# Plachtaa/FAcodec

Measured on NVIDIA B200. Metric: audio_seconds_per_second, higher is better.
Workload: dtype f32 I/O and accumulation; every product is a 3-MMA split of fp32 operands: fp16 hi + 2^11-scaled fp16 lo (22 mantissa bits, register-promoted accumulation) upstream of the VQ, bf16 hi + bf16 lo (16 bits) downstream

## Files before the change

facodec_b200/csrc/conv_tt.cu:

```cuda
#include <cstring>
#include <mutex>

#include "common.cuh"
#include "conv_tc_common.cuh"
#include "kernels.h"

namespace fac {

namespace tc {
constexpr int kThreadsT = 512;
constexpr int kProdT = 192;
constexpr int kStagesT = 4;
constexpr int kABufT = 4;
constexpr int kPfT = 3;
constexpr int kMT = 128;
constexpr int kAccT = 128;
struct SmemT {
    uint64_t b_full[kStagesT];
    uint64_t b_empty[kStagesT];
    uint64_t a_full[kABufT];
    uint64_t a_empty[kABufT];
    uint64_t acc_ready;
    uint64_t acc_free;
    uint32_t tmem_base;
    uint32_t pad;
};
static_assert(sizeof(SmemT) <= kSmemHdr, "SmemT header");
}

__device__ __forceinline__ float sin2_wide(float x) {
    const double kd = rint((double)x * 0.31830988618379067154);
    const float r = (float)fma(-kd, 3.14159265358979323846, (double)x);
    const float r2 = r * r;
    float q = fmaf(r2, 1.60590438368216146e-10f, -2.50521083854417188e-8f);
    q = fmaf(q, r2, 2.75573192239858907e-6f);
    q = fmaf(q, r2, -1.98412698412698413e-4f);
    q = fmaf(q, r2, 8.33333333333333333e-3f);
    q = fmaf(q, r2, -1.66666666666666667e-1f);
    q = fmaf(q * r2, r, r);
    return q * q;
}
__device__ __forceinline__ float4 snake4_w(float4 x, float4 al, float4 ia) {
    const float y0 = al.x * x.x, y1 = al.y * x.y, y2 = al.z * x.z, y3 = al.w * x.w;
    const float m = fmaxf(fmaxf(fabsf(y0), fabsf(y1)), fmaxf(fabsf(y2), fabsf(y3)));
    float4 o;
    if (m > 4096.0f) {
// ... 102 lines not shown
    const int pc = ptid & 3;
    const int r0 = ptid >> 2;
    const bool has_alpha = p.in_alpha != nullptr;
    const bool mufu = p.snake_mufu != 0;
    float4 al = make_float4(0.f, 0.f, 0.f, 0.f), ia = al;
    if (has_alpha) {
        const int j = c * tc::kChunk + pc * 4;
        const int ci = j - (j / p.Cin) * p.Cin;
        al = __ldg(reinterpret_cast<const float4*>(p.in_alpha + ci));
        ia = __ldg(reinterpret_cast<const float4*>(p.in_inv_alpha + ci));
    }
    const uint32_t off0 = ((uint32_t)(pc >> 1) * Rpad + r0) * 16 + (uint32_t)(pc & 1) * 8;
    const float4* __restrict__ st = reinterpret_cast<const float4*>(stage) + ptid;
#pragma unroll
    for (int u = 0; u < NB; ++u) {
        if (r0 + u * RSTEP < R) {
            float4 x4 = st[u * NTHR];
            if (has_alpha) x4 = mufu ? snake4_mufu(x4, al, ia) : snake4_w(x4, al, ia);
            split_store_h(x4, ahi, alo, off0 + u * (RSTEP * 16));
        }
    }
}

template <int ACTT>
__device__ __forceinline__ void epilogue_slab8(float (&v)[8], float bi, float al, float ia, int act, float* __restrict__ yb,
                                               const float* __restrict__ rb, uint32_t off, uint32_t ldy, int nvalid, bool mufu) {
    float r[8];
    if (rb) {
#pragma unroll
        for (int i = 0; i < 8; ++i) r[i] = (i < nvalid) ? rb[off + i * ldy] : 0.f;
    }
#pragma unroll
    for (int i = 0; i < 8; ++i) v[i] += bi;
    if (ACTT == ACT_SNAKE || (ACTT < 0 && act == ACT_SNAKE)) {
        float y[8], m = 0.f;
#pragma unroll
        for (int i = 0; i < 8; ++i) { y[i] = al * v[i]; m = fmaxf(m, fabsf(y[i])); }
        if (m > 4096.0f) {
#pragma unroll
            for (int i = 0; i < 8; ++i) v[i] = fmaf(ia, sin2_wide(y[i]), v[i]);
        } else if (mufu) {
#pragma unroll
            for (int i = 0; i < 8; ++i) v[i] = fmaf(ia, sin2_mufu(y[i]), v[i]);
        } else {
#pragma unroll
            for (int i = 0; i < 8; ++i) v[i] = fmaf(ia, sin2_poly(y[i]), v[i]);
        }
    } else if (ACTT < 0 && act == ACT_TANH) {
#pragma unroll 1
        for (int i = 0; i < 8; ++i) v[i] = tanhf(v[i]);
    } else if (ACTT < 0 && act == ACT_MISH) {
#pragma unroll 1
        for (int i = 0; i < 8; ++i) v[i] = mish_f(v[i]);
    }
    if (rb) {
#pragma unroll
        for (int i = 0; i < 8; ++i) v[i] += r[i];
    }
    if (nvalid >= 8) {
#pragma unroll
        for (int i = 0; i < 8; ++i) yb[off + i * ldy] = v[i];
    } else {
#pragma unroll
        for (int i = 0; i < 8; ++i)
            if (i < nvalid) yb[off + i * ldy] = v[i];
    }
}

__device__ long long g_tt_probe[8];

template <bool PROBE, int ACTT>
__global__ void __launch_bounds__(tc::kThreadsT, 1) conv_tt_kernel(TcConvParams p) {
    using namespace tc;
    extern __shared__ __align__(128) uint8_t smem_raw[];
    SmemT* sm = reinterpret_cast<SmemT*>(smem_raw);
    constexpr int KG = 2;
    const int NT = p.NT;
    const int R = NT + (p.Kr - 1) * p.dil;
    const int Rpad = p.Rpad;
    const uint32_t a_half = (uint32_t)Rpad * 16 * KG;
    constexpr uint32_t w_half = (uint32_t)kMT * 16 * KG;
    uint8_t* a_base = smem_raw + kSmemHdr;
    uint8_t* w_base = a_base + (size_t)kABufT * 2 * a_half;
    const int CT = p.pair ? 2 : 1;
    const uint32_t w_stage = (uint32_t)CT * 2 * w_half;
    uint8_t* stg_base = w_base + (size_t)kStagesT * w_stage;
    constexpr int S = kStagesT;
    const int P = p.promote_every;

    const int tid = threadIdx.x, warp = tid >> 5, lane = tid & 31;
    const int nchunk = p.nchunk, Kr = p.Kr;
    const int gx = (p.Tout + NT - 1) / NT, gy = ((p.Cout + kMT - 1) / kMT) / CT;
    const int ntiles = gx * gy * p.B;
    const int G = (nchunk + P - 1) / P;

    if (tid == 0) {
        for (int i = 0; i < S; ++i) { mbar_init(&sm->b_full[i], 1); mbar_init(&sm->b_empty[i], 1); }
        for (int i = 0; i < kABufT; ++i) { mbar_init(&sm->a_full[i], kProdT); mbar_init(&sm->a_empty[i], 1); }
        mbar_init(&sm->acc_ready, 1);
        mbar_init(&sm->acc_free, 256);
        fence_mbar_init();
    }
    constexpr int kWarpTma = 14, kWarpMma = 15;
    if (warp == kWarpMma) tmem_alloc(&sm->tmem_base, 512);
    tc_fence_before();
    __syncthreads();
    tc_fence_after();
    const uint32_t tmem = sm->tmem_base;

    if (warp >= 8) reg_dec<64>();
    if (warp == kWarpTma) {
        if (lane == 0) {
            int it = 0;
            for (int L = blockIdx.x; L < ntiles; L += gridDim.x) {
                const int ntile = (L % gy) * CT;
                const size_t tile_floats = (size_t)nchunk * Kr * (size_t)(2 * w_half / 4);
                const float* wsrc = p.wblob + (size_t)ntile * tile_floats;
                for (int j = 0; j < nchunk * Kr; ++j, ++it) {
                    const int s = it % S;
                    mbar_wait_park<200>(&sm->b_empty[s], ((it / S) & 1) ^ 1);
                    mbar_arrive_expect_tx(&sm->b_full[s], w_stage);
                    for (int ct = 0; ct < CT; ++ct)
                        bulk_g2s(w_base + (size_t)s * w_stage + (size_t)ct * 2 * w_half, wsrc + (size_t)ct * tile_floats + (size_t)j * (2 * w_half / 4),
                                 2 * w_half, &sm->b_full[s]);
                }
            }
        }
    } else if (warp == kWarpMma) {
        const uint32_t idesc = (1u << 4) | ((uint32_t)(NT >> 3) << 17) | ((128u >> 4) << 24);
        const uint32_t tmem_u = __shfl_sync(0xffffffffu, tmem, 0);
        const uint32_t a_base16 = __shfl_sync(0xffffffffu, smem_u32(a_base), 0) >> 4;
        const uint32_t w_base16 = __shfl_sync(0xffffffffu, smem_u32(w_base), 0) >> 4;
        const uint32_t a_lbo16 = (uint32_t)Rpad, w_lbo16 = (uint32_t)kMT;
        const uint32_t a_half16 = a_half >> 4, w_half16 = w_half >> 4;
        const uint32_t d0 = tmem_u, d1 = tmem_u + 256u;
        int it = 0, cg = 0, gg = 0;
        const bool mprobe = PROBE && blockIdx.x == 3;
        long long w_a = 0, w_b = 0, w_acc = 0, tq = 0;
        for (int L = blockIdx.x; L < ntiles; L += gridDim.x) {
            for (int g = 0; g < G; ++g, ++gg) {
                if (mprobe) tq = clock64();
                mbar_wait(&sm->acc_free, (gg & 1) ^ 1);
                if (mprobe) w_acc += clock64() - tq;
                tc_fence_after();
                const int c_begin = g * P, c_end = (c_begin + P < nchunk) ? c_begin + P : nchunk;
                for (int c = c_begin; c < c_end; ++c, ++cg) {
                    const int buf = cg % kABufT;
                    if (mprobe) tq = clock64();
                    mbar_wait(&sm->a_full[buf], (cg / kABufT) & 1);
                    if (mprobe) w_a += clock64() - tq;
                    const uint32_t x_hi = a_base16 + (uint32_t)buf * 2 * a_half16;
                    const uint32_t x_lo = x_hi + a_half16;
                    for (int tap = 0; tap < Kr; ++tap, ++it) {
                        const int s = it % S;
                        if (mprobe) tq = clock64();
                        mbar_wait(&sm->b_full[s], (it / S) & 1);
                        if (mprobe) w_b += clock64() - tq;
                        tc_fence_after();
                        const uint32_t row_off = (uint32_t)(tap * p.dil);
                        const uint32_t first0 = ((c - c_begin) | tap) != 0, first1 = (g | (c - c_begin) | tap) != 0;
                        for (int ct = 0; ct < CT; ++ct) {
                            const uint32_t w_hi = w_base16 + (uint32_t)s * (w_stage >> 4) + (uint32_t)ct * 2 * w_half16;
                            const uint32_t w_lo = w_hi + w_half16;
                            const uint32_t dc = (uint32_t)ct * 128u;
                            umma_bf16(d0 + dc, desc_u(w_hi, w_lbo16), desc_u(x_hi + row_off, a_lbo16), idesc, first0);
                            umma_bf16(d1 + dc, desc_u(w_hi, w_lbo16), desc_u(x_lo + row_off, a_lbo16), idesc, first1);
                            umma_bf16(d1 + dc, desc_u(w_lo, w_lbo16), desc_u(x_hi + row_off, a_lbo16), idesc, 1u);
                        }
                        umma_commit(&sm->b_empty[s]);
                    }
                    umma_commit(&sm->a_empty[buf]);
                }
                umma_commit(&sm->acc_ready);
            }
        }
        if (mprobe && lane == 0) { g_tt_probe[2] = w_a; g_tt_probe[3] = w_b; g_tt_probe[4] = w_acc; }
    } else if (warp >= 8) {
        const int wtid = tid - 256;
        const PadMap pm = PadMap::make(p.Tin, p.pad_left_s, p.pad_right_s, p.reflect);
        const bool pprobe = PROBE && blockIdx.x == 3 && wtid == 0;
        const long long t_start = pprobe ? clock64() : 0;
        long long w_ae = 0, tq = 0;
        struct Cur { int L, c, t0, vrow0; bool interior; const float* xb; };
        auto setup = [&](Cur& k) {
            k.t0 = ((k.L / gy) % gx) * NT;
            k.xb = p.x + (size_t)(k.L / (gx * gy)) * p.x_bstride;
            k.vrow0 = k.t0 - p.PLr;
            k.interior = k.vrow0 >= 0 && (k.vrow0 + R) * p.vf <= p.Tin && k.t0 + NT <= p.Tout && R <= 7 * (kProdT / 4);
        };
        auto advance = [&](Cur& k) {
            if (++k.c == nchunk) { k.c = 0; k.L += gridDim.x; if (k.L < ntiles) setup(k); }
        };
        Cur pf{(int)blockIdx.x, 0, 0, 0, false, nullptr}, cs = pf;
        if (pf.L < ntiles) { setup(pf); cs = pf; }
        constexpr uint32_t kStageBytes = 7u * kProdT * 16u;
#pragma unroll 1
        for (int i = 0; i < kPfT - 1; ++i) {
// ... 9 lines not shown
            if (pf.L < ntiles) {
                if (pf.interior) stage_chunk_interior<kProdT, 7>(p, pf.xb, pf.c, pf.vrow0, R, stg_base + (size_t)((cg + kPfT - 1) % kPfT) * kStageBytes, wtid);
                advance(pf);
            }
            cp_async_commit_tt();
            cp_async_wait_tt<kPfT - 1>();
            const int buf = cg % kABufT;
            uint8_t* ahi = a_base + (size_t)buf * 2 * a_half;
            if (pprobe) tq = clock64();
            mbar_wait_park<200>(&sm->a_empty[buf], ((cg / kABufT) & 1) ^ 1);
            if (pprobe) w_ae += clock64() - tq;
            if (cs.interior) transform_chunk_interior<kProdT, 7>(p, cs.c, R, Rpad, stg_base + (size_t)(cg % kPfT) * kStageBytes, ahi, ahi + a_half, wtid);
            else produce_chunk_edge<kProdT>(p, pm, cs.xb, cs.c, cs.t0, R, Rpad, ahi, ahi + a_half, wtid);
            fence_proxy_async();
            mbar_arrive(&sm->a_full[buf]);
            advance(cs);
        }
        cp_async_wait_tt<0>();
        if (pprobe) { g_tt_probe[0] = clock64() - t_start; g_tt_probe[1] = w_ae; }
    } else {
        reg_inc<192>();
        const int q = warp & 3;
        const int half = warp >> 2;
        int split = ((NT / 2 + 15) / 16) * 16;
        if (split > NT) split = NT;
        const int mycol0 = CT == 2 ? half * 128 : (half ? split : 0);
        const int mytime0 = CT == 2 ? 0 : mycol0;
        const int mycols = CT == 2 ? NT : (half ? NT - split : split);
        const int act = p.out_act;
        int gg = 0;
        const bool aprobe = PROBE && blockIdx.x == 3 && tid == 0;
        long long w_ar = 0, t_dr = 0, t_ep = 0, tq = 0;
        for (int L = blockIdx.x; L < ntiles; L += gridDim.x) {
            const int ntile = (L % gy) * CT + (CT == 2 ? half : 0);
            const int t0 = ((L / gy) % gx) * NT;
            const int b = L / (gx * gy);
            const int co = ntile * kMT + q * 32 + lane;
            const bool co_ok = co < p.Cout;
            float acc[kAccT];
#pragma unroll
            for (int i = 0; i < kAccT; ++i) acc[i] = 0.f;
            for (int g = 0; g < G; ++g, ++gg) {
                if (aprobe) tq = clock64();
                mbar_wait_park<100>(&sm->acc_ready, gg & 1);
                if (aprobe) { long long n = clock64(); w_ar += n - tq; tq = n; }
                tc_fence_after();
                const uint32_t tb0 = tmem + ((uint32_t)(q * 32) << 16) + (uint32_t)mycol0;
#pragma unroll
                for (int grp = 0; grp < kAccT / 16; ++grp) {
                    if (grp * 16 < mycols) {
                        uint32_t v[16];
                        tmem_ld16(tb0 + grp * 16, v);
#pragma unroll
                        for (int i = 0; i < 16; ++i) acc[grp * 16 + i] += __uint_as_float(v[i]);
                    }
                }
                if (g == G - 1) {
#pragma unroll
                    for (int grp = 0; grp < kAccT / 16; ++grp) {
                        if (grp * 16 < mycols) {
                            uint32_t v[16];
                            tmem_ld16(tb0 + 256u + grp * 16, v);
#pragma unroll
                            for (int i = 0; i < 16; ++i) acc[grp * 16 + i] = fmaf(__uint_as_float(v[i]), kLoUnscale, acc[grp * 16 + i]);
                        }
                    }
                }
                tc_fence_before();
                mbar_arrive(&sm->acc_free);
                if (aprobe) t_dr += clock64() - tq;
            }
            if (aprobe) tq = clock64();
            float* __restrict__ yb = p.y + (size_t)b * p.y_bstride + co;
            const float* __restrict__ rb = p.res ? p.res + (size_t)b * p.y_bstride + co : nullptr;
            float bi = 0.f, al = 0.f, ia = 0.f;
            if (co_ok) {
                if (p.bias) bi = __ldg(p.bias + co);
                if (act == ACT_SNAKE) { al = __ldg(p.out_alpha + co); ia = __ldg(p.out_inv_alpha + co); }
            }
            const int tbeg = t0 + mytime0;
            const uint32_t ldy = (uint32_t)p.ldy;
#pragma unroll 1
            for (int sl = 0; sl * 8 < mycols; ++sl) {
                float v[8];
#define FAC_SLAB(S0) _Pragma("unroll") for (int i = 0; i < 8; ++i) v[i] = acc[(S0) + i];
                switch (sl) {
                    case 0: FAC_SLAB(0) break;
                    case 1: FAC_SLAB(8) break;
                    case 2: FAC_SLAB(16) break;
                    case 3: FAC_SLAB(24) break;
                    case 4: FAC_SLAB(32) break;
                    case 5: FAC_SLAB(40) break;
                    case 6: FAC_SLAB(48) break;
                    case 7: FAC_SLAB(56) break;
                    case 8: FAC_SLAB(64) break;
                    case 9: FAC_SLAB(72) break;
                    case 10: FAC_SLAB(80) break;
                    case 11: FAC_SLAB(88) break;
                    case 12: FAC_SLAB(96) break;
                    case 13: FAC_SLAB(104) break;
                    case 14: FAC_SLAB(112) break;
                    default: FAC_SLAB(120) break;
                }
#undef FAC_SLAB
                const int ts = tbeg + sl * 8;
                const int nvalid = co_ok ? p.Tout - ts : 0;
                if (nvalid > 0) epilogue_slab8<ACTT>(v, bi, al, ia, act, yb, rb, (uint32_t)ts * ldy, ldy, nvalid, p.snake_mufu != 0);
            }
            if (aprobe) t_ep += clock64() - tq;
        }
        if (aprobe) { g_tt_probe[5] = w_ar; g_tt_probe[6] = t_dr; g_tt_probe[7] = t_ep; }
    }
    tc_fence_before();
    __syncthreads();
    if (warp == kWarpMma) tmem_dealloc(tmem, 512);
}

int g_tt_pair_ok = 1;

bool tt_conv_plan(TcConvParams& p) {
    if ((p.Cin % 4) != 0 || ((p.Cin * p.vf) % tc::kChunk) != 0 || p.Cout < 1) return false;
    p.tt = 1; p.promoted = 1; p.f16x2 = 1; p.bf16 = 0; p.fused = 0;
    p.N = tc::kMT; p.MT = 1;
    p.nchunk = p.Cin * p.vf / tc::kChunk;
    p.nchunk2 = 0;
    int NT = 256;
    if (p.Tout > 0) {
        auto padded = [&](int nt) { return (long long)((p.Tout + nt - 1) / nt) * nt; };
        long long best = padded(256);
        for (int cand = 240; cand >= 128; cand -= 16)
            if (padded(cand) * 10 < best * 9) { best = padded(cand); NT = cand; }
    }
    const int ntile_co = (p.Cout + tc::kMT - 1) / tc::kMT;
    p.pair = (g_tt_pair_ok && p.Kr <= 3 && ntile_co >= 2 && ntile_co % 2 == 0) ? 1 : 0;
    if (p.pair) {
        NT = 128;
        if (p.Tout > 0) {
            auto padded = [&](int nt) { return (long long)((p.Tout + nt - 1) / nt) * nt; };
            long long best = padded(128);
            for (int cand = 112; cand >= 64; cand -= 16)
                if (padded(cand) * 10 < best * 9) { best = padded(cand); NT = cand; }
        }
    }
    p.NT = NT;
    p.promote_every = 48 / p.Kr < 1 ? 1 : 48 / p.Kr;
    int R = NT + (p.Kr - 1) * p.dil, Rpad = R;
    while (Rpad % 8 != 2) ++Rpad;
    p.Rpad = Rpad;
    p.tmem_cols = 512;
    p.stagesB = tc::kStagesT;
    const size_t a_bytes = (size_t)tc::kABufT * 2 * Rpad * 16 * 2, w_bytes = (size_t)(p.pair ? 2 : 1) * tc::kStagesT * 2 * tc::kMT * 16 * 2;
    p.smem_bytes = tc::kSmemHdr + a_bytes + w_bytes + (size_t)tc::kPfT * 7 * tc::kProdT * 16;
    return p.smem_bytes <= 225 * 1024;
}

size_t tt_blob_floats(const TcConvParams& p) {
    return (size_t)((p.Cout + tc::kMT - 1) / tc::kMT) * p.nchunk * p.Kr * 2 * 2 * tc::kMT * 4;
}

void tt_pack_blob(const TcConvParams& p, const float* wp, int ldw, float* blob) {
    const int Cw = p.Cin * p.vf;
    uint16_t* ob = reinterpret_cast<uint16_t*>(blob);
    size_t o16 = 0;
    const int ntile = (p.Cout + tc::kMT - 1) / tc::kMT;
    for (int nt = 0; nt < ntile; ++nt)
        for (int c = 0; c < p.nchunk; ++c)
            for (int tap = 0; tap < p.Kr; ++tap)
                for (int hl = 0; hl < 2; ++hl)
                    for (int k8 = 0; k8 < 2; ++k8)
                        for (int n = 0; n < tc::kMT; ++n)
                            for (int e = 0; e < 8; ++e) {
                                const int co = nt * tc::kMT + n;
                                const int kk = tap * Cw + c * tc::kChunk + k8 * 8 + e;
                                const float w = co < p.Cout ? wp[(size_t)kk * ldw + co] : 0.f;
                                __half hi = __float2half_rn(w);
                                __half v = hl == 0 ? hi : __float2half_rn((w - __half2float(hi)) * 2048.0f);
// ... 9 lines not shown
namespace {
struct DevCfgT { bool done = false; int sm_count = 0; };
DevCfgT g_devcfg_t[64];
std::mutex g_devcfg_t_mu;
}

cudaError_t launch_conv_tt(const TcConvParams& p, cudaStream_t st) {
    if (p.Tout <= 0 || p.B <= 0) return cudaSuccess;
    int dev = 0;
    cudaError_t e = cudaGetDevice(&dev);
    if (e != cudaSuccess) return e;
    if (dev < 0 || dev >= 64) return cudaErrorInvalidDevice;
    int sm_count;
    {
        std::lock_guard<std::mutex> lk(g_devcfg_t_mu);
        DevCfgT& d = g_devcfg_t[dev];
        if (!d.done) {
            const int cap = 225 * 1024;
            e = cudaFuncSetAttribute(conv_tt_kernel<false, ACT_NONE>, cudaFuncAttributeMaxDynamicSharedMemorySize, cap);
            if (e == cudaSuccess) e = cudaFuncSetAttribute(conv_tt_kernel<false, ACT_SNAKE>, cudaFuncAttributeMaxDynamicSharedMemorySize, cap);
            if (e == cudaSuccess) e = cudaFuncSetAttribute(conv_tt_kernel<false, -1>, cudaFuncAttributeMaxDynamicSharedMemorySize, cap);
            if (e == cudaSuccess) e = cudaFuncSetAttribute(conv_tt_kernel<true, ACT_NONE>, cudaFuncAttributeMaxDynamicSharedMemorySize, cap);
            if (e == cudaSuccess) e = cudaFuncSetAttribute(conv_tt_kernel<true, ACT_SNAKE>, cudaFuncAttributeMaxDynamicSharedMemorySize, cap);
            if (e != cudaSuccess) return e;
            if (cudaDeviceGetAttribute(&d.sm_count, cudaDevAttrMultiProcessorCount, dev) != cudaSuccess || d.sm_count <= 0) d.sm_count = 148;
            d.done = true;
        }
        sm_count = d.sm_count;
    }
    const long long gx = (p.Tout + p.NT - 1) / p.NT, gy = ((p.Cout + tc::kMT - 1) / tc::kMT) / (p.pair ? 2 : 1);
    const long long ntiles = gx * gy * p.B;
    if (ntiles > 0x7fffffffLL) return cudaErrorInvalidValue;
    const unsigned nctas = (unsigned)(ntiles < sm_count ? ntiles : sm_count);
    if (g_tt_probe_on && p.out_act == ACT_NONE) conv_tt_kernel<true, ACT_NONE><<<dim3(nctas), tc::kThreadsT, p.smem_bytes, st>>>(p);
    else if (g_tt_probe_on && p.out_act == ACT_SNAKE) conv_tt_kernel<true, ACT_SNAKE><<<dim3(nctas), tc::kThreadsT, p.smem_bytes, st>>>(p);
    else if (p.out_act == ACT_NONE) conv_tt_kernel<false, ACT_NONE><<<dim3(nctas), tc::kThreadsT, p.smem_bytes, st>>>(p);
    else if (p.out_act == ACT_SNAKE) conv_tt_kernel<false, ACT_SNAKE><<<dim3(nctas), tc::kThreadsT, p.smem_bytes, st>>>(p);
    else conv_tt_kernel<false, -1><<<dim3(nctas), tc::kThreadsT, p.smem_bytes, st>>>(p);
    return cudaGetLastError();
}

}
```

facodec_b200/csrc/engine.cu:

```cuda
#include <cmath>
#include <cstdio>
#include <cstdlib>
#include <cstring>
#include <map>
#include <string>
#include <vector>

#include "../../include/facodec_b200.h"
#include "../../include/facodec_b200_debug.h"
#include "common.cuh"
#include "kernels.h"

using namespace fac;

namespace {

constexpr int HOP = 300;
constexpr int LATENT = 1024;
constexpr int N_FFT = 2048;
constexpr int WIN = 1200;
constexpr int N_BINS = 1025;
constexpr int SPEC_LD = 2052;
constexpr int SPEC_TC_LD = 2176;
constexpr int N_MELS = 80;
// ... 683 lines not shown
    if (!tc_conv_plan(tp)) return false;
    if (c.dry) return true;
    const int k_eff = (r.c7.K - 1) * r.dil + 1;
    tp.x = x; tp.y = y; tp.res = x;
    tp.wblob = c.W(tp.g1f16 ? r.c7.tcw_f16s : (tp.bf16 ? r.c7.tcw16 : r.c7.tcw)); tp.bias = c.W(r.c7.b);
    tp.wblob2 = c.W(tp.bf16 ? r.c1.tcw16 : r.c1.tcw); tp.bias2 = c.W(r.c1.b);
    tp.in_alpha = c.W(r.s1.a); tp.in_inv_alpha = c.W(r.s1.ia);
    tp.out_act = ACT_SNAKE; tp.out_alpha = c.W(r.s2.a); tp.out_inv_alpha = c.W(r.s2.ia);
    tp.B = B; tp.Tin = T; tp.ldx = r.c7.Cin;
    const int pl = causal ? k_eff - 1 : (k_eff - 1) - (k_eff - 1) / 2;
    tp.PLr = pl; tp.pad_left_s = pl; tp.pad_right_s = k_eff - 1 - pl; tp.reflect = 1;
    tp.Tout = T; tp.ldy = r.c7.Cout;
    tp.x_bstride = (size_t)T * r.c7.Cin; tp.y_bstride = (size_t)T * r.c7.Cout;
    double flops = 2.0 * B * T * (double)r.c7.Cout * r.c7.Cin * (r.c7.K + 1);
    double bytes = 4.0 * ((double)B * T * r.c7.Cin * 2 + (double)B * T * r.c7.Cout + (double)(r.c7.K + 1) * r.c7.Cin * r.c7.Cout);
    char det[96];
    snprintf(det, sizeof det, "res.fused C%d K%d d%d T%d", r.c7.Cin, r.c7.K, r.dil, T);
    c.begin("conv_tc", flops, bytes, det);
    c.check(launch_conv_tc(tp, c.st), "res.fused");
    c.end();
    return true;
}

void residual_unit(Ctx& c, const ResW& r, const float* x, float* tmp, float* y, int B, int T, bool causal = true) {
    if (residual_unit_fused(c, r, x, y, B, T, causal)) return;
    ConvOpts o1;
    o1.in_snake = &r.s1;
    o1.out_snake = &r.s2;
    sconv(c, r.c7, x, tmp, B, T, r.dil, 1, o1, "res.conv7", causal);
    ConvOpts o2;
    o2.res = x;
    sconv(c, r.c1, tmp, y, B, T, 1, 1, o2, "res.conv1", causal);
}

struct LstmState { uint32_t* h[2] = {nullptr, nullptr}; float* c[2] = {nullptr, nullptr}; };

void slstm(Ctx& c, const LstmW& L, const float* x, float* y, int B, int T, LstmState* st = nullptr) {
    const int H = L.H;
    float* xg = c.alloc<float>((size_t)B * T * 4 * H);
    float* h1 = c.alloc<float>((size_t)B * T * H);
    float* hT = c.alloc<float>((size_t)2 * H * 32);
    uint32_t* h16 = c.alloc<uint32_t>((size_t)2 * 2 * (H / 2) * 32);
    unsigned int* bar = c.alloc<unsigned int>(64);
    for (int l = 0; l < 2; ++l) {
        const float* in = l == 0 ? x : h1;
        ConvOpts o;
        run_conv(c, L.ih[l], in, xg, 1, B * T, B * T, o, "lstm.ih");
        if (c.dry) continue;
// ... 1416 lines not shown
    tp.x = x; tp.y = y; tp.wblob = d; tp.bias = d + o_b;
    if (in_alpha_host) { tp.in_alpha = d + o_ia; tp.in_inv_alpha = d + o_iia; }
    tp.out_act = act;
    if (out_alpha_host) { tp.out_act = ACT_SNAKE; tp.out_alpha = d + o_oa; tp.out_inv_alpha = d + o_oia; }
    tp.res = res;
    tp.B = B; tp.Tin = Tin; tp.ldx = Cin;
    tp.PLr = pad_left / tp.vf;
    tp.pad_left_s = pad_left; tp.pad_right_s = pad_right; tp.reflect = reflect;
    tp.Tout = Tout; tp.ldy = Cout;
    tp.x_bstride = (size_t)Tin * Cin; tp.y_bstride = (size_t)Tout * Cout;
    e = use_tt ? launch_conv_tt(tp, st) : launch_conv_tc(tp, st);
    if (e == cudaSuccess) e = cudaStreamSynchronize(st);
    cudaFree(d);
    if (e != cudaSuccess) { h->err = std::string("fac_debug_conv_tc: ") + cudaGetErrorString(e); return FAC_ERR_CUDA; }
    return FAC_OK;
}

int fac_debug_resunit(fac_handle* h, const float* x, const float* w7_host, const float* b7_host, const float* w1_host,
                      const float* b1_host, const float* alpha1_host, const float* alpha2_host, int B, int T, int C,
                      int dil, int mode, float* y, void* stream) {
    if (!h || !x || !y || !w7_host || !w1_host) return FAC_ERR_INVALID;
    fac_handle tmp;
    tmp.device = h->device;
    tmp.use_tc = mode == 0 ? 0 : 1;
    tmp.fuse_res = (mode == 2 || mode == 4 || mode == 6) ? 1 : 0;
    tmp.dec_bf16 = mode >= 3;
    tmp.dec_c7_f16 = mode >= 5;
    tmp.tc_occ2 = h->tc_occ2;
    auto put = [&](const char* key, const float* d, std::vector<int64_t> shp) {
        HostTensor t;
        t.shape = shp;
        t.data.assign(d, d + t.numel());
        tmp.host[0][key] = std::move(t);
    };
    put("u.block.0.alpha", alpha1_host, {1, C, 1});
    put("u.block.1.conv.conv.weight", w7_host, {C, C, 7});
    put("u.block.1.conv.conv.bias", b7_host, {C});
    put("u.block.2.alpha", alpha2_host, {1, C, 1});
    put("u.block.3.conv.conv.weight", w1_host, {C, C, 1});
    put("u.block.3.conv.conv.bias", b1_host, {C});
    ResW r;
    try { r = pack_res(&tmp, 0, "u", dil, false); } catch (const PackError& e) { h->err = e.msg; return FAC_ERR_STATE; }
    cudaSetDevice(h->device);
    cudaError_t e = cudaMalloc(&tmp.warena, (tmp.pack.size() + 64) * sizeof(float));
    if (e == cudaSuccess) e = cudaMemcpy(tmp.warena, tmp.pack.data(), tmp.pack.size() * sizeof(float), cudaMemcpyHostToDevice);
    if (e != cudaSuccess) { h->err = cudaGetErrorString(e); cudaGetLastError(); return FAC_ERR_CUDA; }
    cudaStream_t st = (cudaStream_t)stream;
    float* scratch = nullptr;
    e = cudaMalloc(&scratch, sizeof(float) * (size_t)B * T * C);
    int rc = FAC_OK;
    if (e != cudaSuccess) { h->err = cudaGetErrorString(e); rc = FAC_ERR_CUDA; }
    if (rc == FAC_OK) {
        Ctx c{&tmp, st, false};
        residual_unit(c, r, x, scratch, y, B, T);
        rc = finish(&tmp, c);
        cudaError_t e2 = cudaStreamSynchronize(st);
        if (rc == FAC_OK && e2 != cudaSuccess) { tmp.err = cudaGetErrorString(e2); rc = FAC_ERR_CUDA; }
        if (rc == FAC_OK && (mode == 2 || mode == 4 || mode == 6) && tmp.launches != 1) { tmp.err = "fused path not taken for this geometry"; rc = FAC_ERR_UNSUPPORTED; }
    }
    if (rc != FAC_OK) h->err = tmp.err;
    if (scratch) cudaFree(scratch);
    cudaFree(tmp.warena);
    return rc;
}

long long fac_debug_lstm_pack(const float* whh_host, int H, int bf16, float* out, long long capacity_floats, int* info3) {
    if (!whh_host || H <= 0) return FAC_ERR_INVALID;
    fac_handle tmp;
    const char* names[8] = {"weight_ih_l0", "weight_hh_l0", "bias_ih_l0", "bias_hh_l0", "weight_ih_l1", "weight_hh_l1", "bias_ih_l1", "bias_hh_l1"};
    for (int i = 0; i < 8; ++i) {
        HostTensor t;
        const bool mat = (i % 4) < 2;
        if (mat) t.shape = {4 * H, H}; else t.shape = {4 * H};
        if (i == 1) t.data.assign(whh_host, whh_host + (size_t)4 * H * H);
        else t.data.assign(t.numel(), 0.f);
        tmp.host[0][std::string("l.") + names[i]] = std::move(t);
    }
    LstmW L;
    try { L = pack_lstm(&tmp, 0, "l"); } catch (const PackError&) { return FAC_ERR_UNSUPPORTED; }
    if (info3) { info3[0] = L.U; info3[1] = L.G; info3[2] = 4 * L.U; }
    if (bf16 == 2 || bf16 == 3) {
// ... 19 lines not shown
    b.shape = {Cout};
    b.data.assign(Cout, 0.f);
    tmp.host[0]["c.weight"] = std::move(t);
    tmp.host[0]["c.bias"] = std::move(b);
    ConvW c;
    try { c = causal ? pack_convtr(&tmp, 0, "c", stride) : pack_convtr_noncausal(&tmp, 0, "c", stride); }
    catch (const PackError&) { return FAC_ERR_UNSUPPORTED; }
    const long long n = (long long)c.K * Cin * c.Cout;
    if (!out || capacity_floats < n) return n;
    for (int k = 0; k < c.K; ++k)
        for (int ci = 0; ci < Cin; ++ci)
            for (int co = 0; co < c.Cout; ++co) out[((size_t)k * Cin + ci) * c.Cout + co] = tmp.pack[c.w + ((size_t)k * Cin + ci) * c.ldw + co];
    return n;
}

int fac_debug_pad_map(int L, int pad_left, int pad_right, int reflect, int* out, int n) {
    if (!out || L < 0 || pad_left < 0 || pad_right < 0 || n != pad_left + L + pad_right) return FAC_ERR_INVALID;
    const PadMap pm = PadMap::make(L, pad_left, pad_right, reflect);
    for (int i = 0; i < n; ++i) out[i] = pm.src(i - pad_left);
    return FAC_OK;
}

int fac_debug_tc_plan(int Cin, int Cout, int K, int dil, int stride, int Tout, int mode, int occ2_maxn, int* out8) {
    if (!out8 || Cin <= 0 || Cout <= 0 || K <= 0 || dil <= 0 || stride <= 0 || mode < 0 || mode > 6) return FAC_ERR_INVALID;
    TcConvParams tp;
    tp.Cin = Cin; tp.Cout = Cout; tp.Tout = Tout; tp.occ2_maxn = occ2_maxn;
    tp.promoted = (mode == 1 || mode == 3) ? 1 : 0;
    tp.bf16 = (mode == 2 || mode == 4) ? 1 : 0;
    tp.f16x2 = mode == 3 ? 1 : 0;
    tp.fused = (mode == 4 || mode == 5) ? 1 : 0;
    if (stride == 1) { tp.vf = 1; tp.Kr = K; tp.dil = dil; }
    else if (K == 2 * stride && dil == 1) { tp.vf = stride; tp.Kr = 2; tp.dil = 1; }
    else return FAC_ERR_UNSUPPORTED;
    if (mode == 6) {
        tp.promoted = 0; tp.bf16 = 0; tp.f16x2 = 0; tp.fused = 0;
        if (!tt_conv_plan(tp)) return FAC_ERR_UNSUPPORTED;
        out8[0] = tp.N * (tp.pair ? 2 : 1);
        out8[1] = tp.NT; out8[2] = tp.nchunk; out8[3] = tp.stagesB; out8[4] = tp.tmem_cols;
        out8[5] = (int)tp.smem_bytes; out8[6] = tp.Rpad; out8[7] = tp.promote_every;
        return FAC_OK;
    }
    if (!tc_conv_plan(tp)) return FAC_ERR_UNSUPPORTED;
    out8[0] = tp.N; out8[1] = tp.MT; out8[2] = tp.nchunk; out8[3] = tp.stagesB; out8[4] = tp.tmem_cols;
    out8[5] = (int)tp.smem_bytes; out8[6] = tp.Rpad; out8[7] = tp.promote_every;
    return FAC_OK;
}

long long fac_debug_tc_pack(const float* w_host, int Cin, int Cout, int K, int stride, int mode, float* blob_out,
                            long long capacity_floats) {
    if (!w_host || Cin <= 0 || Cout <= 0 || K <= 0 || stride <= 0 || mode < 0 || mode > 4) return FAC_ERR_INVALID;
    TcConvParams tp;
    tp.Cin = Cin; tp.Cout = Cout; tp.dil = 1;
    tp.promoted = (mode == 1 || mode == 3) ? 1 : 0; tp.bf16 = mode == 2 ? 1 : 0; tp.f16x2 = mode == 3 ? 1 : 0;
    if (stride == 1) { tp.vf = 1; tp.Kr = K; }
    else if (K == 2 * stride) { tp.vf = stride; tp.Kr = 2; }
    else return FAC_ERR_UNSUPPORTED;
    const bool use_tt = mode == 4;
    if (use_tt) { tp.promoted = 0; tp.bf16 = 0; tp.f16x2 = 0; }
    if (!(use_tt ? tt_conv_plan(tp) : tc_conv_plan(tp))) return FAC_ERR_UNSUPPORTED;
// ... 123 lines not shown
```

facodec_b200/csrc/kernels.h:

```cpp
#pragma once
#include <cuda_runtime.h>
#include <stdint.h>

namespace fac {

struct ConvParams {
    const float* x = nullptr;
    const float* w = nullptr;
    const float* bias = nullptr;
    const float* in_alpha = nullptr;
    const float* in_inv_alpha = nullptr;
    const float* out_alpha = nullptr;
    const float* out_inv_alpha = nullptr;
    const float* res = nullptr;
    const int* valid_len = nullptr;
    float* y = nullptr;
    int B = 0, Tin = 0, Cin = 0, Tout = 0, Cout = 0;
    int K = 1, dil = 1, stride = 1, pad_left = 0, pad_right = 0, pad_reflect = 0;
    int ldw = 0, ldy = 0, ldx = 0;
    int out_act = 0;
    int y_transposed = 0;
    size_t x_bstride = 0, y_bstride = 0;
};
cudaError_t launch_conv(const ConvParams& p, cudaStream_t st);
// ... 24 lines not shown
    int snake_mufu = 0;
    int fused = 0;
    const float* wblob2 = nullptr;
    const float* bias2 = nullptr;
    int nchunk2 = 0;
    int occ2_maxn = 0;
    int promote_every = 1;
    int N = 0, MT = 0, nchunk = 0, Rpad = 0, stagesB = 0, tmem_cols = 0;
    int cps = 0;
    int tpt = 1, tpt2 = 1;
    int b_slot = 0;
    int R2pad = 0;
    int dbg = 0;
    int ng = 1;
    int wide = 0;
    size_t smem_bytes = 0;
    size_t x_bstride = 0, y_bstride = 0;
};
bool tc_conv_plan(TcConvParams& p);
size_t tc_blob_floats(const TcConvParams& p);
void tc_pack_blob(const TcConvParams& p, const float* wp, int ldw, float* blob);
cudaError_t launch_conv_tc(const TcConvParams& p, cudaStream_t st);
bool tt_conv_plan(TcConvParams& p);
size_t tt_blob_floats(const TcConvParams& p);
void tt_pack_blob(const TcConvParams& p, const float* wp, int ldw, float* blob);
cudaError_t launch_conv_tt(const TcConvParams& p, cudaStream_t st);
extern int g_tc_dbg;
extern int g_tc_slot_issue;
extern int g_tc_groups_ok;
extern int g_tc_wide_ok;
extern int g_tt_pair_ok;
extern int g_tt_probe_on;
cudaError_t tt_read_probe(long long* out8);
cudaError_t tc_read_trace(long long* out80);
cudaError_t tc_read_producer_clocks(long long* out4);
cudaError_t tc_read_phase_clocks(long long* out8);

struct LstmParams {
    const float* xg = nullptr;
    const float* whh_p = nullptr;
    const float* whh_p16 = nullptr;
    int bf16 = 0;
    const uint32_t* whh_p2 = nullptr;
    uint32_t* h16 = nullptr;
    int pass3 = 0;
    uint32_t* state_h = nullptr;
// ... 83 lines not shown
```

Before: 2225.

## Fuse encoder residual unit (k7 conv, snake, 1x1 conv) into one tcgen05 kernel

```diff
diff --git a/facodec_b200/csrc/conv_tt.cu b/facodec_b200/csrc/conv_tt.cu
--- a/facodec_b200/csrc/conv_tt.cu
+++ b/facodec_b200/csrc/conv_tt.cu
@@ -10,7 +10,7 @@
 namespace tc {
 constexpr int kThreadsT = 512;
 constexpr int kProdT = 192;
-constexpr int kStagesT = 4;
+constexpr int kStagesT = 8;
 constexpr int kABufT = 4;
 constexpr int kPfT = 3;
 constexpr int kMT = 128;
@@ -22,6 +22,7 @@
     uint64_t a_empty[kABufT];
     uint64_t acc_ready;
     uint64_t acc_free;
+    uint64_t b2_full;
     uint32_t tmem_base;
     uint32_t pad;
 };
@@ -170,6 +171,35 @@
     }
 }
 
+__device__ __forceinline__ void snake_slab8(float (&v)[8], float al, float ia, bool mufu) {
+    float y[8], m = 0.f;
+#pragma unroll
+    for (int i = 0; i < 8; ++i) { y[i] = al * v[i]; m = fmaxf(m, fabsf(y[i])); }
+    if (m > 4096.0f) {
+#pragma unroll
+        for (int i = 0; i < 8; ++i) v[i] = fmaf(ia, sin2_wide(y[i]), v[i]);
+    } else if (mufu) {
+#pragma unroll
+        for (int i = 0; i < 8; ++i) v[i] = fmaf(ia, sin2_mufu(y[i]), v[i]);
+    } else {
+#pragma unroll
+        for (int i = 0; i < 8; ++i) v[i] = fmaf(ia, sin2_poly(y[i]), v[i]);
+    }
+}
+
+__device__ __forceinline__ void b2_slab8(float (&v)[8], float bi, float al, float ia, uint8_t* hi, uint8_t* lo, bool mufu) {
+#pragma unroll
+    for (int i = 0; i < 8; ++i) v[i] += bi;
+    snake_slab8(v, al, ia, mufu);
+#pragma unroll
+    for (int i = 0; i < 8; ++i) {
+        const __half h = __float2half_rn(v[i]);
+        const __half l = __float2half_rn((v[i] - __half2float(h)) * tc::kLoScale);
+        *reinterpret_cast<__half*>(hi + i * 16) = h;
+        *reinterpret_cast<__half*>(lo + i * 16) = l;
+    }
+}
+
 template <int ACTT>
 __device__ __forceinline__ void epilogue_slab8(float (&v)[8], float bi, float al, float ia, int act, float* __restrict__ yb,
                                                const float* __restrict__ rb, uint32_t off, uint32_t ldy, int nvalid, bool mufu) {
@@ -181,19 +211,7 @@
 #pragma unroll
     for (int i = 0; i < 8; ++i) v[i] += bi;
     if (ACTT == ACT_SNAKE || (ACTT < 0 && act == ACT_SNAKE)) {
-        float y[8], m = 0.f;
-#pragma unroll
-        for (int i = 0; i < 8; ++i) { y[i] = al * v[i]; m = fmaxf(m, fabsf(y[i])); }
-        if (m > 4096.0f) {
-#pragma unroll
-            for (int i = 0; i < 8; ++i) v[i] = fmaf(ia, sin2_wide(y[i]), v[i]);
-        } else if (mufu) {
-#pragma unroll
-            for (int i = 0; i < 8; ++i) v[i] = fmaf(ia, sin2_mufu(y[i]), v[i]);
-        } else {
-#pragma unroll
-            for (int i = 0; i < 8; ++i) v[i] = fmaf(ia, sin2_poly(y[i]), v[i]);
-        }
+        snake_slab8(v, al, ia, mufu);
     } else if (ACTT < 0 && act == ACT_TANH) {
 #pragma unroll 1
         for (int i = 0; i < 8; ++i) v[i] = tanhf(v[i]);
@@ -217,7 +235,7 @@
 
 __device__ long long g_tt_probe[8];
 
-template <bool PROBE, int ACTT>
+template <bool PROBE, int ACTT, bool FUSED = false>
 __global__ void __launch_bounds__(tc::kThreadsT, 1) conv_tt_kernel(TcConvParams p) {
     using namespace tc;
     extern __shared__ __align__(128) uint8_t smem_raw[];
@@ -232,8 +250,10 @@
     uint8_t* w_base = a_base + (size_t)kABufT * 2 * a_half;
     const int CT = p.pair ? 2 : 1;
     const uint32_t w_stage = (uint32_t)CT * 2 * w_half;
-    uint8_t* stg_base = w_base + (size_t)kStagesT * w_stage;
-    constexpr int S = kStagesT;
+    const int S = p.stagesB;
+    uint8_t* stg_base = w_base + (size_t)S * w_stage;
+    uint8_t* b2_base = stg_base + (size_t)kPfT * 7 * kProdT * 16;
+    const uint32_t b2_half = (uint32_t)p.nchunk2 * KG * p.R2pad * 16;
     const int P = p.promote_every;
 
     const int tid = threadIdx.x, warp = tid >> 5, lane = tid & 31;
@@ -247,6 +267,7 @@
         for (int i = 0; i < kABufT; ++i) { mbar_init(&sm->a_full[i], kProdT); mbar_init(&sm->a_empty[i], 1); }
         mbar_init(&sm->acc_ready, 1);
         mbar_init(&sm->acc_free, 256);
+        mbar_init(&sm->b2_full, 256);
         fence_mbar_init();
     }
     constexpr int kWarpTma = 14, kWarpMma = 15;
@@ -258,19 +279,31 @@
 
     if (warp >= 8) reg_dec<64>();
     if (warp == kWarpTma) {
-        if (lane == 0) {
-            int it = 0;
-            for (int L = blockIdx.x; L < ntiles; L += gridDim.x) {
-                const int ntile = (L % gy) * CT;
-                const size_t tile_floats = (size_t)nchunk * Kr * (size_t)(2 * w_half / 4);
-                const float* wsrc = p.wblob + (size_t)ntile * tile_floats;
-                for (int j = 0; j < nchunk * Kr; ++j, ++it) {
-                    const int s = it % S;
+        const bool dupw = CT == 1 && p.Cout <= 64;
+        int it = 0;
+        for (int L = blockIdx.x; L < ntiles; L += gridDim.x) {
+            const int ntile = (L % gy) * CT;
+            const size_t tile_floats = (size_t)nchunk * Kr * (size_t)(2 * w_half / 4);
+            const float* wsrc = p.wblob + (size_t)ntile * tile_floats;
+            const int nst = nchunk * Kr + (FUSED ? p.nchunk2 : 0);
+            for (int j = 0; j < nst; ++j, ++it) {
+                const int s = it % S;
+                const float* src = j < nchunk * Kr ? wsrc + (size_t)j * (2 * w_half / 4) : p.wblob2 + (size_t)(j - nchunk * Kr) * (2 * w_half / 4);
+                uint8_t* dst = w_base + (size_t)s * w_stage;
+                if (lane == 0) {
                     mbar_wait_park<200>(&sm->b_empty[s], ((it / S) & 1) ^ 1);
                     mbar_arrive_expect_tx(&sm->b_full[s], w_stage);
+                }
+                __syncwarp();
+                if (dupw) {
+                    if (lane < 8) {
+                        const int blk = lane >> 1;
+                        bulk_g2s(dst + blk * (kMT * 16) + (lane & 1) * (kMT * 8), reinterpret_cast<const uint8_t*>(src) + blk * (kMT * 16),
+                                 kMT * 8, &sm->b_full[s]);
+                    }
+                } else if (lane == 0) {
                     for (int ct = 0; ct < CT; ++ct)
-                        bulk_g2s(w_base + (size_t)s * w_stage + (size_t)ct * 2 * w_half, wsrc + (size_t)ct * tile_floats + (size_t)j * (2 * w_half / 4),
-                                 2 * w_half, &sm->b_full[s]);
+                        bulk_g2s(dst + (size_t)ct * 2 * w_half, src + (size_t)ct * tile_floats, 2 * w_half, &sm->b_full[s]);
                 }
             }
         }
@@ -282,7 +315,9 @@
         const uint32_t a_lbo16 = (uint32_t)Rpad, w_lbo16 = (uint32_t)kMT;
         const uint32_t a_half16 = a_half >> 4, w_half16 = w_half >> 4;
         const uint32_t d0 = tmem_u, d1 = tmem_u + 256u;
-        int it = 0, cg = 0, gg = 0;
+        const uint32_t b2_base16 = __shfl_sync(0xffffffffu, smem_u32(b2_base), 0) >> 4;
+        const uint32_t b2_lbo16 = (uint32_t)p.R2pad, b2_half16 = b2_half >> 4;
+        int it = 0, cg = 0, gg = 0, tl = 0;
         const bool mprobe = PROBE && blockIdx.x == 3;
         long long w_a = 0, w_b = 0, w_acc = 0, tq = 0;
         for (int L = blockIdx.x; L < ntiles; L += gridDim.x) {
@@ -321,6 +356,28 @@
                 }
                 umma_commit(&sm->acc_ready);
             }
+            if (FUSED) {
+                if (mprobe) tq = clock64();
+                mbar_wait(&sm->b2_full, tl & 1);
+                if (mprobe) w_acc += clock64() - tq;
+                tc_fence_after();
+                for (int c = 0; c < p.nchunk2; ++c, ++it) {
+                    const int s = it % S;
+                    if (mprobe) tq = clock64();
+                    mbar_wait(&sm->b_full[s], (it / S) & 1);
+                    if (mprobe) w_b += clock64() - tq;
+                    tc_fence_after();
+                    const uint32_t w_hi = w_base16 + (uint32_t)s * (w_stage >> 4), w_lo = w_hi + w_half16;
+                    const uint32_t x_hi = b2_base16 + (uint32_t)(c * KG) * b2_lbo16, x_lo = x_hi + b2_half16;
+                    const uint32_t first = c != 0;
+                    umma_bf16(d0, desc_u(w_hi, w_lbo16), desc_u(x_hi, b2_lbo16), idesc, first);
+                    umma_bf16(d1, desc_u(w_hi, w_lbo16), desc_u(x_lo, b2_lbo16), idesc, first);
+                    umma_bf16(d1, desc_u(w_lo, w_lbo16), desc_u(x_hi, b2_lbo16), idesc, 1u);
+                    umma_commit(&sm->b_empty[s]);
+                }
+                umma_commit(&sm->acc_ready);
+                ++tl;
+            }
         }
         if (mprobe && lane == 0) { g_tt_probe[2] = w_a; g_tt_probe[3] = w_b; g_tt_probe[4] = w_acc; }
     } else if (warp >= 8) {
@@ -376,12 +433,15 @@
         reg_inc<192>();
         const int q = warp & 3;
         const int half = warp >> 2;
-        int split = ((NT / 2 + 15) / 16) * 16;
-        if (split > NT) split = NT;
-        const int mycol0 = CT == 2 ? half * 128 : (half ? split : 0);
+        const bool dup = CT == 1 && p.Cout <= 64;
+        const int tparts = dup ? 4 : 2, tpart = dup ? half * 2 + (q >> 1) : half;
+        const int qs = ((NT / tparts + 15) / 16) * 16;
+        const int tb = min(NT, tpart * qs), te = min(NT, tb + qs);
+        const int mycol0 = CT == 2 ? half * 128 : tb;
         const int mytime0 = CT == 2 ? 0 : mycol0;
-        const int mycols = CT == 2 ? NT : (half ? NT - split : split);
-        const int act = p.out_act;
+        const int mycols = CT == 2 ? NT : te - tb;
+        const int act = FUSED ? ACT_NONE : p.out_act;
+        const float* __restrict__ ep_bias = FUSED ? p.bias2 : p.bias;
         int gg = 0;
         const bool aprobe = PROBE && blockIdx.x == 3 && tid == 0;
         long long w_ar = 0, t_dr = 0, t_ep = 0, tq = 0;
@@ -389,7 +449,7 @@
             const int ntile = (L % gy) * CT + (CT == 2 ? half : 0);
             const int t0 = ((L / gy) % gx) * NT;
             const int b = L / (gx * gy);
-            const int co = ntile * kMT + q * 32 + lane;
+            const int co = ntile * kMT + (dup ? (q & 1) : q) * 32 + lane;
             const bool co_ok = co < p.Cout;
             float acc[kAccT];
 #pragma unroll
@@ -420,6 +480,65 @@
                         }
                     }
                 }
+                if (!FUSED || g < G - 1) {
+                    tc_fence_before();
+                    mbar_arrive(&sm->acc_free);
+                }
+                if (aprobe) t_dr += clock64() - tq;
+            }
+            if (FUSED) {
+                if (aprobe) tq = clock64();
+                if (co_ok) {
+                    const float bi = p.bias ? __ldg(p.bias + co) : 0.f;
+                    const float al = __ldg(p.out_alpha + co), ia = __ldg(p.out_inv_alpha + co);
+                    const uint32_t off = ((uint32_t)(co >> 4) * KG + (uint32_t)((co >> 3) & 1)) * p.R2pad * 16 + (uint32_t)(co & 7) * 2 +
+                                         (uint32_t)mytime0 * 16;
+                    uint8_t* hi = b2_base + off;
+#pragma unroll 1
+                    for (int sl = 0; sl * 8 < mycols; ++sl) {
+                        float v[8];
+#define FAC_SLAB(S0) _Pragma("unroll") for (int i = 0; i < 8; ++i) v[i] = acc[(S0) + i];
+                        switch (sl) {
+                            case 0: FAC_SLAB(0) break;
+                            case 1: FAC_SLAB(8) break;
+                            case 2: FAC_SLAB(16) break;
+                            case 3: FAC_SLAB(24) break;
+                            case 4: FAC_SLAB(32) break;
+                            case 5: FAC_SLAB(40) break;
+                            case 6: FAC_SLAB(48) break;
+                            case 7: FAC_SLAB(56) break;
+                            case 8: FAC_SLAB(64) break;
+                            case 9: FAC_SLAB(72) break;
+                            case 10: FAC_SLAB(80) break;
+                            case 11: FAC_SLAB(88) break;
+                            case 12: FAC_SLAB(96) break;
+                            case 13: FAC_SLAB(104) break;
+                            case 14: FAC_SLAB(112) break;
+                            default: FAC_SLAB(120) break;
+                        }
+#undef FAC_SLAB
+                        b2_slab8(v, bi, al, ia, hi + sl * 128, hi + b2_half + sl * 128, p.snake_mufu != 0);
+                    }
+                }
+                fence_proxy_async();
+                tc_fence_before();
+                mbar_arrive(&sm->b2_full);
+                if (aprobe) { long long n = clock64(); t_dr += n - tq; tq = n; }
+                mbar_wait_park<100>(&sm->acc_ready, gg & 1);
+                ++gg;
+                if (aprobe) { long long n = clock64(); w_ar += n - tq; tq = n; }
+                tc_fence_after();
+                const uint32_t tb0 = tmem + ((uint32_t)(q * 32) << 16) + (uint32_t)mycol0;
+#pragma unroll
+                for (int grp = 0; grp < kAccT / 16; ++grp) {
+                    if (grp * 16 < mycols) {
+                        uint32_t v0[16], v1[16];
+                        tmem_ld16(tb0 + grp * 16, v0);
+                        tmem_ld16(tb0 + 256u + grp * 16, v1);
+#pragma unroll
+                        for (int i = 0; i < 16; ++i) acc[grp * 16 + i] = fmaf(__uint_as_float(v1[i]), kLoUnscale, __uint_as_float(v0[i]));
+                    }
+                }
                 tc_fence_before();
                 mbar_arrive(&sm->acc_free);
                 if (aprobe) t_dr += clock64() - tq;
@@ -429,7 +548,7 @@
             const float* __restrict__ rb = p.res ? p.res + (size_t)b * p.y_bstride + co : nullptr;
             float bi = 0.f, al = 0.f, ia = 0.f;
             if (co_ok) {
-                if (p.bias) bi = __ldg(p.bias + co);
+                if (ep_bias) bi = __ldg(ep_bias + co);
                 if (act == ACT_SNAKE) { al = __ldg(p.out_alpha + co); ia = __ldg(p.out_inv_alpha + co); }
             }
             const int tbeg = t0 + mytime0;
@@ -472,40 +591,69 @@
 
 int g_tt_pair_ok = 1;
 
+namespace {
+int tt_pick_nt(int Tout, int nt_max) {
+    int NT = nt_max;
+    if (Tout > 0) {
+        auto padded = [&](int nt) { return (long long)((Tout + nt - 1) / nt) * nt; };
+        long long best = padded(nt_max);
+        for (int cand = nt_max - 16; cand >= nt_max / 2; cand -= 16)
+            if (padded(cand) * 10 < best * 9) { best = padded(cand); NT = cand; }
+    }
+    return NT;
+}
+void tt_size(TcConvParams& p) {
+    int R = p.NT + (p.Kr - 1) * p.dil, Rpad = R;
+    while (Rpad % 8 != 2) ++Rpad;
+    p.Rpad = Rpad;
+    int R2pad = p.NT;
+    while (R2pad % 8 != 2) ++R2pad;
+    p.R2pad = p.fused ? R2pad : 0;
+    const size_t a_bytes = (size_t)tc::kABufT * 2 * Rpad * 16 * 2, w_bytes = (size_t)(p.pair ? 2 : 1) * p.stagesB * 2 * tc::kMT * 16 * 2;
+    const size_t b2_bytes = (size_t)2 * p.nchunk2 * 2 * p.R2pad * 16;
+    p.smem_bytes = tc::kSmemHdr + a_bytes + w_bytes + (size_t)tc::kPfT * 7 * tc::kProdT * 16 + b2_bytes;
+}
+constexpr size_t kSmemCapT = 225 * 1024;
+void tt_fit_stages(TcConvParams& p) {
+    p.stagesB = tc::kStagesT;
+    tt_size(p);
+    while (p.smem_bytes > kSmemCapT && p.stagesB > 4) {
+        --p.stagesB;
+        tt_size(p);
+    }
+}
+}
+
 bool tt_conv_plan(TcConvParams& p) {
     if ((p.Cin % 4) != 0 || ((p.Cin * p.vf) % tc::kChunk) != 0 || p.Cout < 1) return false;
     p.tt = 1; p.promoted = 1; p.f16x2 = 1; p.bf16 = 0; p.fused = 0;
     p.N = tc::kMT; p.MT = 1;
     p.nchunk = p.Cin * p.vf / tc::kChunk;
     p.nchunk2 = 0;
-    int NT = 256;
-    if (p.Tout > 0) {
-        auto padded = [&](int nt) { return (long long)((p.Tout + nt - 1) / nt) * nt; };
-        long long best = padded(256);
-        for (int cand = 240; cand >= 128; cand -= 16)
-            if (padded(cand) * 10 < best * 9) { best = padded(cand); NT = cand; }
-    }
     const int ntile_co = (p.Cout + tc::kMT - 1) / tc::kMT;
     p.pair = (g_tt_pair_ok && p.Kr <= 3 && ntile_co >= 2 && ntile_co % 2 == 0) ? 1 : 0;
-    if (p.pair) {
-        NT = 128;
-        if (p.Tout > 0) {
-            auto padded = [&](int nt) { return (long long)((p.Tout + nt - 1) / nt) * nt; };
-            long long best = padded(128);
-            for (int cand = 112; cand >= 64; cand -= 16)
-                if (padded(cand) * 10 < best * 9) { best = padded(cand); NT = cand; }
-        }
-    }
-    p.NT = NT;
+    p.NT = tt_pick_nt(p.Tout, p.pair ? 128 : 256);
     p.promote_every = 48 / p.Kr < 1 ? 1 : 48 / p.Kr;
-    int R = NT + (p.Kr - 1) * p.dil, Rpad = R;
-    while (Rpad % 8 != 2) ++Rpad;
-    p.Rpad = Rpad;
     p.tmem_cols = 512;
-    p.stagesB = tc::kStagesT;
-    const size_t a_bytes = (size_t)tc::kABufT * 2 * Rpad * 16 * 2, w_bytes = (size_t)(p.pair ? 2 : 1) * tc::kStagesT * 2 * tc::kMT * 16 * 2;
-    p.smem_bytes = tc::kSmemHdr + a_bytes + w_bytes + (size_t)tc::kPfT * 7 * tc::kProdT * 16;
-    return p.smem_bytes <= 225 * 1024;
+    tt_fit_stages(p);
+    return p.smem_bytes <= kSmemCapT;
+}
+
+bool tt_resunit_plan(TcConvParams& p) {
+    if (p.vf != 1 || p.Cin != p.Cout || p.Cout > 64 || !tt_conv_plan(p) || p.pair) return false;
+    p.fused = 1;
+    p.nchunk2 = p.Cout / tc::kChunk;
+    int nt_max = 256;
+    p.stagesB = 4;
+    for (; nt_max >= 64; nt_max -= 16) {
+        p.NT = nt_max;
+        tt_size(p);
+        if (p.smem_bytes <= kSmemCapT) break;
+    }
+    if (nt_max < 64) return false;
+    p.NT = tt_pick_nt(p.Tout, nt_max);
+    tt_fit_stages(p);
+    return true;
 }
 
 size_t tt_blob_floats(const TcConvParams& p) {
@@ -561,6 +709,8 @@
             if (e == cudaSuccess) e = cudaFuncSetAttribute(conv_tt_kernel<false, -1>, cudaFuncAttributeMaxDynamicSharedMemorySize, cap);
             if (e == cudaSuccess) e = cudaFuncSetAttribute(conv_tt_kernel<true, ACT_NONE>, cudaFuncAttributeMaxDynamicSharedMemorySize, cap);
             if (e == cudaSuccess) e = cudaFuncSetAttribute(conv_tt_kernel<true, ACT_SNAKE>, cudaFuncAttributeMaxDynamicSharedMemorySize, cap);
+            if (e == cudaSuccess) e = cudaFuncSetAttribute(conv_tt_kernel<false, ACT_NONE, true>, cudaFuncAttributeMaxDynamicSharedMemorySize, cap);
+            if (e == cudaSuccess) e = cudaFuncSetAttribute(conv_tt_kernel<true, ACT_NONE, true>, cudaFuncAttributeMaxDynamicSharedMemorySize, cap);
             if (e != cudaSuccess) return e;
             if (cudaDeviceGetAttribute(&d.sm_count, cudaDevAttrMultiProcessorCount, dev) != cudaSuccess || d.sm_count <= 0) d.sm_count = 148;
             d.done = true;
@@ -571,7 +721,10 @@
     const long long ntiles = gx * gy * p.B;
     if (ntiles > 0x7fffffffLL) return cudaErrorInvalidValue;
     const unsigned nctas = (unsigned)(ntiles < sm_count ? ntiles : sm_count);
-    if (g_tt_probe_on && p.out_act == ACT_NONE) conv_tt_kernel<true, ACT_NONE><<<dim3(nctas), tc::kThreadsT, p.smem_bytes, st>>>(p);
+    if (p.fused && (p.Cout > tc::kMT || p.pair || !p.wblob2 || !p.out_alpha)) return cudaErrorInvalidValue;
+    if (p.fused && g_tt_probe_on) conv_tt_kernel<true, ACT_NONE, true><<<dim3(nctas), tc::kThreadsT, p.smem_bytes, st>>>(p);
+    else if (p.fused) conv_tt_kernel<false, ACT_NONE, true><<<dim3(nctas), tc::kThreadsT, p.smem_bytes, st>>>(p);
+    else if (g_tt_probe_on && p.out_act == ACT_NONE) conv_tt_kernel<true, ACT_NONE><<<dim3(nctas), tc::kThreadsT, p.smem_bytes, st>>>(p);
     else if (g_tt_probe_on && p.out_act == ACT_SNAKE) conv_tt_kernel<true, ACT_SNAKE><<<dim3(nctas), tc::kThreadsT, p.smem_bytes, st>>>(p);
     else if (p.out_act == ACT_NONE) conv_tt_kernel<false, ACT_NONE><<<dim3(nctas), tc::kThreadsT, p.smem_bytes, st>>>(p);
     else if (p.out_act == ACT_SNAKE) conv_tt_kernel<false, ACT_SNAKE><<<dim3(nctas), tc::kThreadsT, p.smem_bytes, st>>>(p);
diff --git a/facodec_b200/csrc/engine.cu b/facodec_b200/csrc/engine.cu
--- a/facodec_b200/csrc/engine.cu
+++ b/facodec_b200/csrc/engine.cu
@@ -729,8 +729,38 @@
     return true;
 }
 
+bool residual_unit_fused_tt(Ctx& c, const ResW& r, const float* x, float* y, int B, int T, bool causal) {
+    if (c.h->use_tc < 2 || !c.h->fuse_res || !c.h->enc_tt || !r.c7.promoted || !r.c1.promoted || !r.c7.has_tt || !r.c1.has_tt ||
+        r.c7.Cin != r.c7.Cout || r.c1.Cin != r.c7.Cout || r.c1.Cout != r.c7.Cout || r.c1.K != 1 || r.c7.vf != 1)
+        return false;
+    TcConvParams tp;
+    tp.Cin = r.c7.Cin; tp.Cout = r.c7.Cout; tp.vf = 1; tp.Kr = r.c7.K; tp.dil = r.dil; tp.Tout = T;
+    if (!tt_resunit_plan(tp)) return false;
+    if (c.dry) return true;
+    const int k_eff = (r.c7.K - 1) * r.dil + 1;
+    tp.x = x; tp.y = y; tp.res = x;
+    tp.wblob = c.W(r.c7.tcw_tt); tp.bias = c.W(r.c7.b);
+    tp.wblob2 = c.W(r.c1.tcw_tt); tp.bias2 = c.W(r.c1.b);
+    tp.in_alpha = c.W(r.s1.a); tp.in_inv_alpha = c.W(r.s1.ia);
+    tp.out_act = ACT_SNAKE; tp.out_alpha = c.W(r.s2.a); tp.out_inv_alpha = c.W(r.s2.ia);
+    tp.snake_mufu = c.h->enc_mufu;
+    tp.B = B; tp.Tin = T; tp.ldx = r.c7.Cin;
+    const int pl = causal ? k_eff - 1 : (k_eff - 1) - (k_eff - 1) / 2;
+    tp.PLr = pl; tp.pad_left_s = pl; tp.pad_right_s = k_eff - 1 - pl; tp.reflect = 1;
+    tp.ldy = r.c7.Cout;
+    tp.x_bstride = (size_t)T * r.c7.Cin; tp.y_bstride = (size_t)T * r.c7.Cout;
+    double flops = 2.0 * B * T * (double)r.c7.Cout * r.c7.Cin * (r.c7.K + 1);
+    double bytes = 4.0 * ((double)B * T * r.c7.Cin * 2 + (double)B * T * r.c7.Cout + (double)(r.c7.K + 1) * r.c7.Cin * r.c7.Cout);
+    char det[96];
+    snprintf(det, sizeof det, "res.fused C%d K%d d%d T%d", r.c7.Cin, r.c7.K, r.dil, T);
+    c.begin("conv_tt", flops, bytes, det);
+    c.check(launch_conv_tt(tp, c.st), "res.fused_tt");
+    c.end();
+    return true;
+}
+
 void residual_unit(Ctx& c, const ResW& r, const float* x, float* tmp, float* y, int B, int T, bool causal = true) {
-    if (residual_unit_fused(c, r, x, y, B, T, causal)) return;
+    if (c.vq_critical ? residual_unit_fused_tt(c, r, x, y, B, T, causal) : residual_unit_fused(c, r, x, y, B, T, causal)) return;
     ConvOpts o1;
     o1.in_snake = &r.s1;
     o1.out_snake = &r.s2;
@@ -2193,10 +2223,12 @@
     if (!h || !x || !y || !w7_host || !w1_host) return FAC_ERR_INVALID;
     fac_handle tmp;
     tmp.device = h->device;
-    tmp.use_tc = mode == 0 ? 0 : 1;
-    tmp.fuse_res = (mode == 2 || mode == 4 || mode == 6) ? 1 : 0;
-    tmp.dec_bf16 = mode >= 3;
-    tmp.dec_c7_f16 = mode >= 5;
+    if (mode < 0 || mode > 8) { h->err = "fac_debug_resunit: mode out of range"; return FAC_ERR_INVALID; }
+    const bool enc = mode >= 7, fused = mode == 2 || mode == 4 || mode == 6 || mode == 8;
+    tmp.use_tc = mode == 0 ? 0 : (enc ? 2 : 1);
+    tmp.fuse_res = fused ? 1 : 0;
+    tmp.dec_bf16 = mode >= 3 && !enc;
+    tmp.dec_c7_f16 = mode >= 5 && !enc;
     tmp.tc_occ2 = h->tc_occ2;
     auto put = [&](const char* key, const float* d, std::vector<int64_t> shp) {
         HostTensor t;
@@ -2211,7 +2243,7 @@
     put("u.block.3.conv.conv.weight", w1_host, {C, C, 1});
     put("u.block.3.conv.conv.bias", b1_host, {C});
     ResW r;
-    try { r = pack_res(&tmp, 0, "u", dil, false); } catch (const PackError& e) { h->err = e.msg; return FAC_ERR_STATE; }
+    try { r = pack_res(&tmp, 0, "u", dil, enc); } catch (const PackError& e) { h->err = e.msg; return FAC_ERR_STATE; }
     cudaSetDevice(h->device);
     cudaError_t e = cudaMalloc(&tmp.warena, (tmp.pack.size() + 64) * sizeof(float));
     if (e == cudaSuccess) e = cudaMemcpy(tmp.warena, tmp.pack.data(), tmp.pack.size() * sizeof(float), cudaMemcpyHostToDevice);
@@ -2223,11 +2255,12 @@
     if (e != cudaSuccess) { h->err = cudaGetErrorString(e); rc = FAC_ERR_CUDA; }
     if (rc == FAC_OK) {
         Ctx c{&tmp, st, false};
+        c.vq_critical = enc;
         residual_unit(c, r, x, scratch, y, B, T);
         rc = finish(&tmp, c);
         cudaError_t e2 = cudaStreamSynchronize(st);
         if (rc == FAC_OK && e2 != cudaSuccess) { tmp.err = cudaGetErrorString(e2); rc = FAC_ERR_CUDA; }
-        if (rc == FAC_OK && (mode == 2 || mode == 4 || mode == 6) && tmp.launches != 1) { tmp.err = "fused path not taken for this geometry"; rc = FAC_ERR_UNSUPPORTED; }
+        if (rc == FAC_OK && fused && tmp.launches != 1) { tmp.err = "fused path not taken for this geometry"; rc = FAC_ERR_UNSUPPORTED; }
     }
     if (rc != FAC_OK) h->err = tmp.err;
     if (scratch) cudaFree(scratch);
@@ -2293,7 +2326,7 @@
 }
 
 int fac_debug_tc_plan(int Cin, int Cout, int K, int dil, int stride, int Tout, int mode, int occ2_maxn, int* out8) {
-    if (!out8 || Cin <= 0 || Cout <= 0 || K <= 0 || dil <= 0 || stride <= 0 || mode < 0 || mode > 6) return FAC_ERR_INVALID;
+    if (!out8 || Cin <= 0 || Cout <= 0 || K <= 0 || dil <= 0 || stride <= 0 || mode < 0 || mode > 7) return FAC_ERR_INVALID;
     TcConvParams tp;
     tp.Cin = Cin; tp.Cout = Cout; tp.Tout = Tout; tp.occ2_maxn = occ2_maxn;
     tp.promoted = (mode == 1 || mode == 3) ? 1 : 0;
@@ -2303,9 +2336,9 @@
     if (stride == 1) { tp.vf = 1; tp.Kr = K; tp.dil = dil; }
     else if (K == 2 * stride && dil == 1) { tp.vf = stride; tp.Kr = 2; tp.dil = 1; }
     else return FAC_ERR_UNSUPPORTED;
-    if (mode == 6) {
+    if (mode == 6 || mode == 7) {
         tp.promoted = 0; tp.bf16 = 0; tp.f16x2 = 0; tp.fused = 0;
-        if (!tt_conv_plan(tp)) return FAC_ERR_UNSUPPORTED;
+        if (!(mode == 7 ? tt_resunit_plan(tp) : tt_conv_plan(tp))) return FAC_ERR_UNSUPPORTED;
         out8[0] = tp.N * (tp.pair ? 2 : 1);
         out8[1] = tp.NT; out8[2] = tp.nchunk; out8[3] = tp.stagesB; out8[4] = tp.tmem_cols;
         out8[5] = (int)tp.smem_bytes; out8[6] = tp.Rpad; out8[7] = tp.promote_every;
diff --git a/facodec_b200/csrc/kernels.h b/facodec_b200/csrc/kernels.h
--- a/facodec_b200/csrc/kernels.h
+++ b/facodec_b200/csrc/kernels.h
@@ -70,6 +70,7 @@
 void tc_pack_blob(const TcConvParams& p, const float* wp, int ldw, float* blob);
 cudaError_t launch_conv_tc(const TcConvParams& p, cudaStream_t st);
 bool tt_conv_plan(TcConvParams& p);
+bool tt_resunit_plan(TcConvParams& p);
 size_t tt_blob_floats(const TcConvParams& p);
 void tt_pack_blob(const TcConvParams& p, const float* wp, int ldw, float* blob);
 cudaError_t launch_conv_tt(const TcConvParams& p, cudaStream_t st);
```

Result: slower. 2191, median of 6 (-1.5%).
